# rrwick/Autocycler

Hardware: AMD Instinct MI355X
Metric: Mbp/sec through compress->unitig GFA (k=51) (higher is better)
Workload: dtype u64

## Files before the change

### autocycler_amd/csrc/device_prims.hpp

```cpp
#pragma once

namespace ac {

#ifdef AC_EMU
inline u64 state_load(const u64* p) {
    struct Seen { const u64* p; u64 v; u32 n; };
    static thread_local Seen seen[1024];
    Seen& e = seen[wv::tid() & 1023u];
    const u64 v = *p;
    if (e.p == p && e.v == v) { if (++e.n > (1u << 20)) { e.n = 0; throw DeviceError("lockstep emulation: a look-back waits for a tile state that is never published"); } }
    else { e.p = p; e.v = v; e.n = 0; }
    return v;
}
inline void state_store(u64* p, u64 v) { *p = v; }
#else
__device__ inline u64 state_load(const u64* p) { return __hip_atomic_load(p, __ATOMIC_RELAXED, __HIP_MEMORY_SCOPE_AGENT); }
__device__ inline void state_store(u64* p, u64 v) { __hip_atomic_store(p, v, __ATOMIC_RELAXED, __HIP_MEMORY_SCOPE_AGENT); }
#endif

AC_HD int prim_popc64(u64 x) {
#if defined(__HIP_DEVICE_COMPILE__)
    return __popcll(x);
#else
    return __builtin_popcountll(x);
// ... 38 lines not shown
            AC_HIP_CHECK(hipStreamSynchronize(0));
            if (want != cap) { if (words) (void)hipFree(words); AC_HIP_CHECK(hipMalloc((void**)&words, want * 8)); }
            AC_HIP_CHECK(hipMemset(words, 0, want * 8));
#endif
            cap = want; epoch = 0; tickets = 0;
        }
        *epoch_out = ++epoch;
        *ticket_base = tickets;
        tickets += tiles;
    }
};
enum { CTX_SCANPOOL = 7 };
inline ScanPool& scan_pool() { return ctx_object<ScanPool>(CTX_SCANPOOL); }

template <class T, int OP, bool INCL>
AC_KERNEL void __launch_bounds__(256) scan_kernel(const T* in, T* out, u64 n, u64* pool, u64 epoch, u64 ticket_base) {
    AC_SHARED u64 s_wave[4];
    AC_SHARED u64 s_prefix;
    AC_SHARED u64 s_tile;
    u64* state = pool + 1;
    const unsigned tid = wv::tid();
    const int lane = wv::lane(), wave = (int)(tid >> 6);
    if (tid == 0) s_tile = atomic_add64(&pool[0], 1) - ticket_base;
    wv::block_sync();
    const u64 tile = s_tile;
    const u64 base = tile * SCAN_TILE + (u64)tid * SCAN_ITEMS;
    alignas(16) T v[SCAN_ITEMS];
    if (base + SCAN_ITEMS <= n && (((uintptr_t)(in + base)) & 15u) == 0) {
        const PrimV16* p = (const PrimV16*)(in + base);
        PrimV16* q = (PrimV16*)v;
#pragma unroll
        for (u32 j = 0; j < SCAN_ITEMS * sizeof(T) / 16; j++) q[j] = p[j];
    } else {
#pragma unroll
        for (u32 j = 0; j < SCAN_ITEMS; j++) v[j] = base + j < n ? in[base + j] : (T)0;
    }
    u64 tsum = 0;
#pragma unroll
    for (u32 j = 0; j < SCAN_ITEMS; j++) tsum = scan_op<OP>(tsum, (u64)v[j]);
    u64 incl = tsum;
// ... 28 lines not shown
        }
        if (lane == 0) s_prefix = excl;
    }
    wv::block_sync();
    u64 run = scan_op<OP>(s_prefix, wave_off);
    {
        const u64 before = wave_shfl_up64(incl, 1);
        if (lane > 0) run = scan_op<OP>(run, before);
    }
    alignas(16) T o[SCAN_ITEMS];
#pragma unroll
    for (u32 j = 0; j < SCAN_ITEMS; j++) {
        const u64 nxt = scan_op<OP>(run, (u64)v[j]);
        o[j] = (T)(INCL ? nxt : run);
        run = nxt;
    }
    if (base + SCAN_ITEMS <= n && (((uintptr_t)(out + base)) & 15u) == 0) {
        PrimV16* q = (PrimV16*)(out + base);
        const PrimV16* p = (const PrimV16*)o;
#pragma unroll
        for (u32 j = 0; j < SCAN_ITEMS * sizeof(T) / 16; j++) q[j] = p[j];
    } else {
#pragma unroll
        for (u32 j = 0; j < SCAN_ITEMS; j++) if (base + j < n) out[base + j] = o[j];
    }
}
template <class T, int OP, bool INCL> inline void scan_launch(const T* in, T* out, size_t n, stream_t s) {
    if (!n) return;
    if (s != 0) throw DeviceError("scan: stream 0 only (the state pool's tickets are stream-ordered)");
    const u64 tiles = (n + SCAN_TILE - 1) / SCAN_TILE;
    u64 epoch = 0, ticket_base = 0;
    ScanPool& pool = scan_pool();
    pool.take(tiles, &epoch, &ticket_base);
    launch_wave_kernel(scan_kernel<T, OP, INCL>, tiles, s, in, out, (u64)n, pool.words, epoch, ticket_base);
}
inline void inclusive_scan_u32(const u32* in, u32* out, size_t n, stream_t s = 0) { scan_launch<u32, SCAN_ADD, true>(in, out, n, s); }
inline void inclusive_max_scan_u32(const u32* in, u32* out, size_t n, stream_t s = 0) { scan_launch<u32, SCAN_MAX, true>(in, out, n, s); }
inline void exclusive_scan_u32(const u32* in, u32* out, size_t n, stream_t s = 0) { scan_launch<u32, SCAN_ADD, false>(in, out, n, s); }
inline void exclusive_scan_u64(const u64* in, u64* out, size_t n, stream_t s = 0) { scan_launch<u64, SCAN_ADD, false>(in, out, n, s); }

static const u32 RS_ITEMS = 8, RS_TILE = 256 * RS_ITEMS, RS_MAX_PASSES = 8;
static const int RS_LB = 16;
template <int UNUSED> AC_KERNEL void __launch_bounds__(256) radix_hist_kernel(const u64* keys, u64 n, int passes, int begin_bit, int end_bit, u32* hist) {
    AC_SHARED u32 s_hist[RS_MAX_PASSES * 256];
    const unsigned tid = wv::tid();
    for (int i = (int)tid; i < passes * 256; i += 256) s_hist[i] = 0;
    wv::block_sync();
    const u64 base = (u64)wv::bid() * RS_TILE;
    for (u32 j = 0; j < RS_ITEMS; j++) {
        const u64 i = base + (u64)j * 256 + tid;
// ... 228 lines not shown
```

### autocycler_amd/csrc/device_rt.hpp

```cpp
#pragma once
#include <cstdio>
#include <cstdlib>
#include <cstring>
#include <stdexcept>
#include <string>
#include <vector>
#include <algorithm>

#include <mutex>
#include <time.h>
#include <unistd.h>

#include "kmer_ops.hpp"
#include "graph_types.hpp"
#include "wave_rt.hpp"

#ifndef AC_EMU
#include <hip/hip_runtime.h>
#endif

namespace ac {

struct DeviceError : std::runtime_error { using std::runtime_error::runtime_error; };
struct NeedExactPositions {};
// ... 464 lines not shown
    if (s == 0) flush_fills();
    if (use_mailbox() && bytes <= Mailbox::CAP) {
        MailItem it{d, (u32)bytes, 0};
        Mailbox::get().fetch(&it, &h, 1, s);
        return;
    }
    static const bool use_scratch = getenv("AC_NO_PINNED_SCRATCH") == nullptr;
    if (use_scratch && bytes <= (64 << 10)) {
        void* p = pinned_scratch(bytes);
        rt_counters().readbacks++;
        AC_HIP_CHECK(hipMemcpyAsync(p, d, bytes, hipMemcpyDeviceToHost, s));
        AC_HIP_CHECK(hipStreamSynchronize(s));
        memcpy(h, p, bytes);
        return;
    }
#endif
    copy_d2h_async(h, d, bytes, s);
#ifndef AC_EMU
    AC_HIP_CHECK(hipStreamSynchronize(s));
#endif
}
class ReadBatch {
  public:
    void add(void* h, const void* d, size_t bytes) { if (bytes) items_.push_back(Item{h, d, bytes}); }
    void run(stream_t s = 0) {
#ifdef AC_EMU
        for (auto& it : items_) memcpy(it.h, it.d, it.bytes);
        (void)s;
#else
        size_t total = 0;
        for (auto& it : items_) total += (it.bytes + 63) & ~(size_t)63;
        if (total == 0) return;
        if (s == 0) flush_fills();
        if (use_mailbox() && total <= Mailbox::CAP && items_.size() <= (size_t)MAIL_MAX_ITEMS) {
            MailItem mi[MAIL_MAX_ITEMS]; void* dst[MAIL_MAX_ITEMS];
            size_t o = 0;
            for (size_t i = 0; i < items_.size(); i++) { mi[i] = MailItem{items_[i].d, (u32)items_[i].bytes, (u32)o}; dst[i] = items_[i].h; o += (items_[i].bytes + 63) & ~(size_t)63; }
            Mailbox::get().fetch(mi, dst, (int)items_.size(), s);
            items_.clear();
            return;
        }
// ... 193 lines not shown
    for (u64 b0 = 0; b0 < blocks; b0 += 0xFFFFFFu)
        wv::launch_kernel(+[](const F* g, u64 nn, u64 base) { const u64 tid = base + (u64)wv::bid() * 256 + wv::tid(); (*g)(tid, tid < nn); },
                          (unsigned)std::min<u64>(0xFFFFFFu, blocks - b0), 256u, fp, n, b0 * 256);
#else
    const u64 blocks = (n + 255) / 256;
    if (s == 0) flush_fills();
    if (debug_launch()) debug_launch_note<F>(n, false);
    for (u64 b0 = 0; b0 < blocks; b0 += MAX_LAUNCH_BLOCKS) {
        rt_counters().launches++;
        hipLaunchKernelGGL(functor_kernel_full<F>, dim3((unsigned)std::min(MAX_LAUNCH_BLOCKS, blocks - b0)), dim3(256), 0, s, n, f, b0 * 256);
        AC_HIP_CHECK(hipGetLastError());
    }
    if (debug_launch()) debug_launch_note<F>(n, true);
#endif
}
template <class K, class... A> void launch_wave_kernel_sized(K kernel, u64 blocks, unsigned threads, stream_t s, A... args) {
    if (blocks == 0) return;
    if (blocks > 0xFFFFFFULL) throw DeviceError("grid too large");
#ifdef AC_EMU
    (void)s;
    wv::launch_kernel(kernel, (unsigned)blocks, threads, args...);
#else
    if (s == 0) flush_fills();
    rt_counters().launches++;
    hipLaunchKernelGGL(kernel, dim3((unsigned)blocks), dim3(threads), 0, s, args...);
    AC_HIP_CHECK(hipGetLastError());
#endif
}
template <class K, class... A> void launch_wave_kernel(K kernel, u64 blocks, stream_t s, A... args) { launch_wave_kernel_sized(kernel, blocks, 256u, s, args...); }
AC_D u32 wave_alloc32(u32* counter, u32 amount) {
// ... 21 lines not shown
```

### autocycler_amd/csrc/graph_impl.hpp

```cpp
#pragma once
#include "graph_build.hpp"

#include <chrono>
#include <cmath>
#include <map>
#include <string>
#include <algorithm>
#include <atomic>
#include <thread>
#include <functional>
#include <condition_variable>
#include <mutex>
#include <fcntl.h>
#include <unistd.h>
#if defined(__x86_64__)
#include <immintrin.h>
#endif

#include "device_rt.hpp"

namespace ac {

static double now_s() {
    return std::chrono::duration<double>(std::chrono::steady_clock::now().time_since_epoch()).count();
// ... 269 lines not shown
    bool shard_degree_flags;
    bool insert_adaptive;
    u64 insert_growth;
    u64 insert_waves_target;
    bool renum_two_pass;
    u32 renum_max_group;
    u32 path_chunk_env;
    long upload_threads_env;
    bool debug_arena;
    bool degree_diag;
    int multi_transport;
    int multi_fragments;
    int multi_tail;
    u64 trim_batch_bytes;
    u64 resolve_batch_bytes;
    static Knobs read() {
        Knobs k;
        k.minkey_variant = [&]() -> int { const char* e = getenv("AC_MINKEY_VARIANT"); return e ? atoi(e) : -1; }();
        k.path_copy = [&]() -> int { const char* e = getenv("AC_PATH_COPY"); return e ? (atoi(e) != 0 ? 1 : 0) : 2; }();
        k.run_piece = [&]() -> u64 { const char* e = getenv("AC_RUN_PIECE"); const long v = e ? atol(e) : 0; return v > 0 ? (u64)v : 4096; }();
        k.pos_cap = [&]() -> u32 { const char* e = getenv("AC_POS_CAP"); const long v = e ? atol(e) : 65536; return v < 0 ? 0u : (u32)std::min<long>(v, 0x3FFFFFFF); }();
        k.path_filter = [&]() -> bool { const char* e = getenv("AC_PATH_FILTER"); return e ? atoi(e) != 0 : true; }();
        k.host_remap_mode = [&]() -> int { const char* e = getenv("AC_HOST_REMAP"); return e ? (atoi(e) == 2 ? 2 : (atoi(e) != 0 ? 1 : 0)) : -1; }();
        k.remap_block = [&]() -> u32 { const char* e = getenv("AC_REMAP_BLOCK"); int v = e ? atoi(e) : 4096; v = v < 64 ? 64 : (v > 65536 ? 65536 : v); return (u32)(v & ~63); }();
        k.minkey_prefix_bases = [&]() -> int { const char* e = getenv("AC_MINKEY_PREFIX_BASES"); int v = e ? atoi(e) : 31; return v < 1 ? 1 : (v > 31 ? 31 : v); }();
        k.seed_prefix_sort = [&]() -> bool { const char* e = getenv("AC_SEED_PREFIX_SORT"); return e ? atoi(e) != 0 : true; }();
        k.seed_max_group = [&]() -> u32 { const char* e = getenv("AC_SEED_MAX_GROUP"); int v = e ? atoi(e) : 1024; return (u32)(v < 1 ? 1 : v); }();
        k.seed_prefix_bits = [&]() -> int { const char* e = getenv("AC_SEED_PREFIX_BITS"); if (!e) return 0; int v = atoi(e); return v < 1 ? 1 : (v > 64 ? 64 : v); }();
        k.degree_region_cap = [&]() -> u32 { const char* e = getenv("AC_DEGREE_REGION_CAP"); int v = e ? atoi(e) : 0; return (u32)(v < 0 ? 0 : v); }();
        k.upload_direct_mode = [&]() -> int { const char* e = getenv("AC_UPLOAD_DIRECT"); return e ? (atoi(e) != 0 ? 1 : 0) : -1; }();
// ... 21 lines not shown
        k.shard_degree_flags = [&]() -> bool { const char* e = getenv("AC_SHARD_DEGREE_FLAGS"); return e ? atoi(e) != 0 : true; }();
        k.insert_adaptive = [&]() -> bool { const char* e = getenv("AC_INSERT_ADAPT"); return e ? atoi(e) != 0 : true; }();
        k.insert_growth = [&]() -> u64 { const char* e = getenv("AC_INSERT_GROWTH"); long x = e ? atol(e) : 2; return (u64)(x < 2 ? 2 : x); }();
        k.insert_waves_target = [&]() -> u64 { const char* e = getenv("AC_INSERT_WAVES"); long x = e ? atol(e) : 16384; return (u64)(x < 1024 ? 1024 : x); }();
        k.renum_two_pass = [&]() -> bool { const char* e = getenv("AC_RENUM_TWO_PASS"); return e && atoi(e) != 0; }();
        k.renum_max_group = [&]() -> u32 { const char* e = getenv("AC_RENUM_MAX_GROUP"); int v = e ? atoi(e) : 64; return (u32)(v < 1 ? 1 : (v > 64 ? 64 : v)); }();
        k.path_chunk_env = [&]() -> u32 { const char* e = getenv("AC_PATH_CHUNK"); if (!e) return 0; int v = atoi(e); return (u32)(v < 64 ? 64 : (v > 4096 ? 4096 : v)); }();
        k.upload_threads_env = [&]() -> long { const char* e = getenv("AC_UPLOAD_THREADS"); return e ? atol(e) : 24; }();
        k.debug_arena = [&]() -> bool { return getenv("AC_DEBUG_ARENA") != nullptr; }();
        k.degree_diag = [&]() -> bool { return getenv("AC_DEGREE_DIAG") != nullptr; }();
        k.multi_transport = [&]() -> int { const char* e = getenv("AC_MULTI_TRANSPORT"); return !e ? 0 : (!strcmp(e, "host") ? 1 : (!strcmp(e, "rccl") ? 2 : 0)); }();
        k.multi_fragments = [&]() -> int { const char* e = getenv("AC_MULTI_FRAGMENTS"); return e && !strcmp(e, "bytes") ? 1 : 0; }();
        k.multi_tail = [&]() -> int { const char* e = getenv("AC_MULTI_TAIL"); return e && !strcmp(e, "replicated") ? 1 : 0; }();
        k.trim_batch_bytes = [&]() -> u64 { const char* e = getenv("AC_TRIM_BATCH_BYTES"); const long long v = e ? atoll(e) : 0; return v > 0 ? (u64)v : (u64)4 << 30; }();
        k.resolve_batch_bytes = [&]() -> u64 { const char* e = getenv("AC_RESOLVE_BATCH_BYTES"); const long long v = e ? atoll(e) : 0; return v > 0 ? (u64)v : (u64)1 << 30; }();
        return k;
    }
};
const Knobs& knobs();
void knobs_refresh();

[[maybe_unused]] static int minkey_variant() { return knobs().minkey_variant; }
[[maybe_unused]] static int path_copy() { return knobs().path_copy; }
[[maybe_unused]] static bool path_copy_pays(u64 n_text, u32 assemblies, u32 k, double r2) {
    const double A = (double)std::max<u32>(assemblies, 1);
    const double entries = (double)n_text * std::min(1.0, 2.0 * A * r2 / (double)k);
    const double saving = entries * 53e-12 * std::max(0.0, 1.0 - 2.0 / A), cost = 0.25e-3 + 0.3e-12 * (double)n_text;
    return saving > 1.5 * cost;
}
[[maybe_unused]] static u64 run_piece() { return knobs().run_piece; }
// ... 147 lines not shown
    void begin(BuildTimings* t) {
        tm = t; t_begin = t0 = now_s();
        rt_counters() = RtCounters();
        host_remap_allowed = false;
        counters.alloc(8); counters.fill_bytes(0);
        sort_flags.alloc(2); sort_flags.fill_bytes(0);
    }
    void check_sizes(const PackedText& t) const {
        if (t.n_text >= POS_MASK) throw DeviceError("input too large for 40-bit text positions");
        if (t.n_seqs == 0 || t.n_text < (u64)k + 2) throw DeviceError("no sequences");
    }
    template <int W> void insert(const PackedText& t, u32 hint, DBuf<u64>* slots_out, u64* cap_out, u64* n_distinct_out, DBuf<u64>* bm_out, bool want_sib = false);
    DBuf<u64> sflags;
    DBuf<u64> runs; DBuf<u32> run_count; u64 run_rows = 0, run_rows_cap = 0;
    DBuf<u64> loc_bm; DBuf<u32> loc_wprefix; bool local_insert_of_shard = false;
    struct CopyPlan { bool ok = false; u64 R = 0, NW = 0, Rb = 0; DBuf<RunRec> rr; DBuf<u32> rseq; DBuf<u64> wfirst, w_begin, w_end; DBuf<u32> w_gap; } cplan;
    void occupancy_bitmap(const DBuf<u64>& sl, u64 c, DBuf<u64>* occ_out, const u64* sflags_in, u64* sib_out, stream_t s = 0);
    DBuf<u64> occ;
    DBuf<u64> sib;
    DBuf<u64> sibn; bool sib_pending = false;
    DBuf<u32> kcontrib, pend, pidx; u64 n_pending = 0, n_first = 0;
    DBuf<u64> endset, endset_bloom; u64 endset_mask = 0;
    u32 n_owners = 1, my_owner = 0;
    void* upload_done = nullptr; u64 upload_avail = 0; bool upload_pending = false;
    struct UploadJob {
#ifndef AC_EMU
        const std::vector<SeqView>* seqs = nullptr;
        std::vector<uint64_t> off;
        uint32_t k = 0; u64 n = 0, CH = 0, SUB = 0, n_chunks = 0, slot_bytes = 0; int NSLOT = 0, dev = 0;
        hipStream_t up = nullptr, pk = nullptr;
        u64* d_bits = nullptr;
// ... 136 lines not shown
```

### autocycler_amd/csrc/graph_stages.hip

```cpp
#include "graph_impl.hpp"

namespace ac {

template <int W>
void GraphBuilder::Impl::insert(const PackedText& pt, u32 hint, DBuf<u64>* slots_out, u64* cap_out, u64* n_distinct_out, DBuf<u64>* bm_out, bool want_sib) {
    TextCtx t = pt.ctx((int)k);
    const u64 p_end_all = pt.n_text - (u64)k + 1;
    if (hint == 0) hint = 1;
    u64 est = pt.n_bases / hint;
    u64 c = next_pow2(std::max<u64>(1024, est * 3 + 4096));
    if (&pt == &uni && distinct_upper) {
        const u64 mine = distinct_upper / std::max<u32>(n_owners, 1) + distinct_upper / (8 * (u64)std::max<u32>(n_owners, 1)) + 4096;
        c = next_pow2(std::max<u64>(1024, mine * 10 / 7));
    }
    if (c > next_pow2(pt.n_bases * 2 + 1024)) c = next_pow2(pt.n_bases * 2 + 1024);
    const int shift = table_shift() >= 0 ? table_shift() : (c > (1ULL << 25) ? 0 : 1);
    c <<= shift;
    struct CapMemo { u64 n_text = 0, cap = 0; u32 k = 0; int shift = -2; u32 owners = 0; };
    static thread_local CapMemo memo[4]; static thread_local unsigned memo_next = 0;
    const u32 memo_owners = (&pt == &uni) ? n_owners : 1u;
    for (const CapMemo& m : memo)
        if (pt.n_text == m.n_text && k == m.k && m.shift == table_shift() && m.owners == memo_owners && m.cap > c) c = m.cap;
    const int copy_mode = (&pt == &loc && (want_sib || (local_insert_of_shard && shard_path_copy()))) ? path_copy() : 0;
    bool want_runs = false;
// ... 439 lines not shown
    std::vector<u64> h_first = to_host(first, n_shards);
    u64 end = n_queries;
    for (u32 o = n_shards; o-- > 0;) {
        if (h_first[o] == ~0ULL) { counts_host[o] = 0; continue; }
        counts_host[o] = end - h_first[o];
        end = h_first[o];
    }
}
template <int W> void GraphBuilder::Impl::answer_queries(const u64* d_keys, u64 n, u64* d_out) {
    launch(n, AnswerFunctor<W>{G->ctx((int)k), graph_table(), d_keys, d_out});
}

template <int W> bool GraphBuilder::Impl::walk_copy_prepare(u32 PC, const Novel& nv_text) {
    TextCtx t = loc.ctx((int)k);
    cplan = CopyPlan();
    const Arena::Mark mk = Arena::device().mark();
    DBuf<u32> rfirst(run_rows + 1);
    exclusive_scan_u32(run_count.ptr(), rfirst.ptr(), run_rows + 1);
    const u64 R0 = read_scalar(rfirst.ptr() + run_rows);
    if (R0 == 0 || R0 >= 0xFFFFFFF0ULL) { Arena::device().rewind(mk); return false; }
    DBuf<RunRec> sorted(R0);
    launch(run_rows * RUN_ROW, RunGatherFunctor{runs.ptr(), run_count.ptr(), rfirst.ptr(), sorted.ptr()});
    DBuf<u32> ok(R0 + 1), at(R0 + 1); DBuf<u64> covered(1, true); DBuf<u32> overlap(1, true);
    ok.fill_bytes(0);
    DBuf<RunRec> fixed(R0); DBuf<u32> fseq(R0);
    launch(R0, RunFilterFunctor{sorted.ptr(), fixed.ptr(), R0, nv_text, loc.n_text, ok.ptr(), covered.ptr(), t, overlap.ptr(), run_piece(), fseq.ptr()});
    exclusive_scan_u32(ok.ptr(), at.ptr(), R0 + 1);
    const u64 Rb = R0 + loc.n_text / run_piece() + 1;
    CopyPlan& c = cplan;
    c.rr.alloc(Rb); c.rseq.alloc(Rb);
    launch(R0, RunCompactFunctor{fixed.ptr(), ok.ptr(), at.ptr(), c.rr.ptr(), run_piece(), fseq.ptr(), c.rseq.ptr(), nv_text, loc.n_text});
    DBuf<u64> gw(Rb + 2);
    c.wfirst.alloc(Rb + 2);
    launch(Rb + 2, GapWalkersFunctor{c.rr.ptr(), at.ptr() + R0, loc.n_text, PC, gw.ptr()});
    exclusive_scan_u64(gw.ptr(), c.wfirst.ptr(), Rb + 2);
    u64 h_cov = 0, NW = 0; u32 h_R = 0, h_overlap = 0;
    { ReadBatch rb; rb.add(&h_cov, covered.ptr(), 8); rb.add(&h_R, at.ptr() + R0, 4); rb.add(&h_overlap, overlap.ptr(), 4); rb.add(&NW, c.wfirst.ptr() + (Rb + 1), 8); rb.run(); }
    const u64 R = h_R;
    if (knobs().debug_arena) fprintf(stderr, "path copy: %llu runs on the list, %llu pieces usable, covering %llu of %llu positions, %llu walkers\n", (unsigned long long)R0, (unsigned long long)R, (unsigned long long)h_cov, (unsigned long long)loc.n_text, (unsigned long long)NW);
    if (R == 0 || h_overlap || h_cov * 2 < loc.n_text || NW == 0 || NW >= 0xFFFFFFF0ULL) {
        cplan = CopyPlan();
        Arena::device().rewind(mk);
        return false;
    }
    c.w_begin.alloc(NW); c.w_end.alloc(NW); c.w_gap.alloc(NW);
    launch(NW, WalkerRangeFunctor{c.rr.ptr(), R, loc.n_text, PC, c.wfirst.ptr(), c.w_begin.ptr(), c.w_end.ptr(), c.w_gap.ptr()});
    c.R = R; c.NW = NW; c.Rb = Rb; c.ok = true;
    return true;
}
template <int W> void GraphBuilder::Impl::walk_copy_finish(u32 PC) {
    TextCtx t = loc.ctx((int)k), g = G->ctx((int)k);
    Table tb = graph_table();
    Novel nv{bm.ptr(), wprefix.ptr()};
    UnitigCtx uc{head.ptr(), scan.ptr(), rank.ptr(), uorient.ptr(), ustart.ptr(), ulen.ptr(), U, N};
    CopyPlan& c = cplan;
    const u64 R = c.R, NW = c.NW;
    DBuf<u64> wcount(NW + 1), woff(NW + 1);
    const u64 n_slots = ((NW + 63) / 64) * 64 * PC;
    DBuf<int32_t> stage(n_slots); DBuf<u16> stage_off(n_slots);
    DBuf<u32> seq_tid(loc.n_seqs), seq_j(loc.n_seqs);
    wcount.fill_bytes(0);
    const bool filter = maybe_dest_valid;
    walk_tables(filter);
    walked_plain = false;
    DBuf<V16> uinfo(U);
    launch(U, WalkInfoFunctor{uc, filter ? maybe_dest.ptr() : nullptr, uinfo.ptr()});
    launch(NW, PathWalkFunctor<W>{t, g, tb, nv, uc, uinfo.ptr(), wl_text.ptr(), PC, stage.ptr(), wcount.ptr(), seq_tid.ptr(), seq_j.ptr(),
                                 depth_u.ptr(), minpos_fwd_u.ptr(), minpos_rev_u.ptr(), counters.ptr() + 4, filter ? maybe_dest.ptr() : nullptr,
                                 pos_cap_now, 0, walk_answers, NW, c.w_begin.ptr(), c.w_end.ptr(), stage_off.ptr(), nullptr, nullptr});
    exclusive_scan_u64(wcount.ptr(), woff.ptr(), NW + 1);
    const u64 NE = read_scalar(woff.ptr() + NW);
    DBuf<int32_t> ent(NE); DBuf<u64> ent_pos(NE), ent_end(NE); DBuf<u8> ent_want(NE); DBuf<u32> ent_gap(NE);
    launch_full(NW, WalkCompactFunctor{stage.ptr(), stage_off.ptr(), wcount.ptr(), woff.ptr(), c.w_begin.ptr(), c.w_gap.ptr(), PC, NW, uinfo.ptr(),
                                       ent.ptr(), ent_pos.ptr(), ent_end.ptr(), ent_want.ptr(), ent_gap.ptr()});
    DBuf<u64> ra(R), rcnt(R + 1), seg(2 * R + 2), segoff(2 * R + 2); DBuf<u32> cov(NE + 1), copies(NE + 1);
    cov.fill_bytes(0);
    launch(R, RunRangeFunctor{c.rr.ptr(), ent_pos.ptr(), ent_end.ptr(), NE, ra.ptr(), rcnt.ptr(), cov.ptr()});
    launch(2 * R + 2, SegCountFunctor{c.wfirst.ptr(), woff.ptr(), rcnt.ptr(), R, seg.ptr()});
    exclusive_scan_u64(seg.ptr(), segoff.ptr(), 2 * R + 2);
    inclusive_scan_u32(cov.ptr(), copies.ptr(), NE + 1);
    n_ent = read_scalar(segoff.ptr() + (2 * R + 1));
    if (knobs().debug_arena) {
        std::vector<u64> h = to_host(rcnt, R); u64 mx = 0, sum = 0, big = 0, hist[8] = {0};
        for (u64 v : h) { mx = std::max(mx, v); sum += v; if (v > 256) big++; int b = 0; while ((32ull << b) < v && b < 7) b++; hist[b]++; }
        fprintf(stderr, "path copy: %llu pieces, entries per piece: max %llu, mean %.1f, %llu above 256; hist(<=32,64,128,..): %llu %llu %llu %llu %llu %llu %llu %llu\n", (unsigned long long)R, (unsigned long long)mx, (double)sum / (double)R, (unsigned long long)big,
                (unsigned long long)hist[0], (unsigned long long)hist[1], (unsigned long long)hist[2], (unsigned long long)hist[3], (unsigned long long)hist[4], (unsigned long long)hist[5], (unsigned long long)hist[6], (unsigned long long)hist[7]);
    }
    ent_val.alloc(n_ent);
    int32_t* const out_ptr = ent_val.ptr();
    launch(NE, GapOutFunctor{ent.ptr(), ent_gap.ptr(), woff.ptr(), c.wfirst.ptr(), segoff.ptr(), copies.ptr(), out_ptr, depth_u.ptr()});
    launch_full(R * 32, RunOutFunctor<32, 1>{c.rr.ptr(), R, ra.ptr(), rcnt.ptr(), segoff.ptr(), ent.ptr(), ent_pos.ptr(), ent_end.ptr(), uinfo.ptr(),
                                             ent_want.ptr(), t, c.rseq.ptr(), minpos_fwd_u.ptr(), minpos_rev_u.ptr(), out_ptr, pos_cap_now});
    launch(loc.n_seqs, PathOffCopyFunctor{seq_tid.ptr(), seq_j.ptr(), woff.ptr(), c.wfirst.ptr(), c.w_gap.ptr(), segoff.ptr(), path_off.ptr()});
    tm->n_path_entries = n_ent;
    tm->path_runs_copied = R; tm->path_entries_walked = NE;
    copy_h2d(path_off.ptr() + loc.n_seqs, &n_ent, 8);
    launch(loc.n_seqs, PathEndsFunctor{ent_val.ptr(), path_off.ptr(), fs0.ptr(), fe0.ptr(), rank.ptr(), uorient.ptr()});
    walk_to_seed_order();
}

template <int W> void GraphBuilder::Impl::walk() {
// ... 70 lines not shown
```

### autocycler_amd/csrc/kernels_paths.inc

```
AC_HD u32 idx_of(int32_t v) { return (u32)(v < 0 ? -v : v) - 1; }
struct MaybeDestFunctor {
    const int32_t* links; u8* maybe;
    AC_HD static u64 row(int32_t v) { return ((u64)((u32)(v < 0 ? -v : v) - 1) * 2 + (v > 0 ? 0 : 1)) * 5; }
    AC_HD void operator()(u64 idx) const {
        const u32 x = (u32)(idx >> 1);
        const bool inputs = (idx & 1) == 0;
        const int32_t xnum = (int32_t)x + 1;
        const u64 mine = row(inputs ? -xnum : xnum);
        u32 n = 0;
        bool ok = true;
        for (int c = 0; c < 5; c++) {
            int32_t p = links[mine + (u64)c];
            if (p == 0) continue;
            n++;
            int32_t other = inputs ? -p : p;
            const u64 theirs = row(inputs ? other : -other);
            u32 m = 0; int32_t only = 0;
            for (int d = 0; d < 5; d++) { int32_t q = links[theirs + (u64)d]; if (q != 0) { m++; only = q; } }
            if (!(m == 1 && only == (inputs ? xnum : -xnum))) ok = false;
            if ((u32)(other < 0 ? -other : other) - 1 == x) ok = false;
        }
        maybe[idx] = (ok && n >= 2) ? 1 : 0;
    }
};
// ... 165 lines not shown
        for (u32 o0 = 0; o0 < total; o0 += 64) {
            const u32 o = o0 + (u32)lane;
            int lo = 0;
#pragma unroll
            for (int step = 32; step; step >>= 1) {
                const int cand = lo + step;
                const u32 v = (u32)wv::shfl((int)rel, cand & 63);
                if (cand < 64 && v <= o) lo = cand;
            }
            const u32 start = (u32)wv::shfl((int)rel, lo);
            if (o < total) ent_val[base + o] = rows[(u64)(o - start) * 64 + (u64)lo];
        }
    }
};
struct RunRec { u64 p; u64 n; u64 q; };
struct RunGatherFunctor {
    const u64* runs; const u32* count; const u32* rfirst; RunRec* out;
    AC_HD void operator()(u64 tid) const {
        const u64 row = tid / RUN_ROW; const u32 i = (u32)(tid % RUN_ROW);
        if (i >= count[row]) return;
        const u64* rec = runs + 3 * tid;
        out[(u64)rfirst[row] + i] = RunRec{rec[0], rec[1], rec[2]};
    }
};
AC_HD bool run_piece_good(const Novel& nv, u64 n_text, const RunRec& x, u64 d, u64 n) {
    const bool same = (x.q >> 63) != 0;
    const u64 q = x.q & ~(1ULL << 63);
    if (!same && q < d + n - 1) return false;
    const u64 qlo = same ? q + d : q - d + 1 - n, qhi = qlo + n;
    if (qhi > n_text) return false;
    return (u64)(novel_rank(nv, qhi) - novel_rank(nv, qlo)) == n;
}
struct RunFilterFunctor {
    const RunRec* runs; RunRec* fixed; u64 n_runs; Novel nv; u64 n_text; u32* ok; u64* covered; TextCtx t; u32* overlap; u64 piece; u32* fseq;
    AC_D void operator()(u64 r) const {
        RunRec x = runs[r];
        const bool same = (x.q >> 63) != 0;
        u64 q = x.q & ~(1ULL << 63);
        u32 lo = 0;
        {
            u32 hi = t.n_seqs;
            while (hi - lo > 1) { u32 mid = lo + ((hi - lo) >> 1); if (t.seq_off[mid] <= x.p) lo = mid; else hi = mid; }
            if (t.n_seqs && t.seq_off[lo] == x.p && x.n > 0) {
                x.p += 1; x.n -= 1; q = same ? q + 1 : q - 1;
                x.q = q | ((u64)(same ? 1 : 0) << 63);
            }
        }
        fixed[r] = x; fseq[r] = lo;
        if (r > 0 && runs[r - 1].p + runs[r - 1].n > runs[r].p) atomic_or32(overlap, 1u);
// ... 13 lines not shown
        if (!ok[r]) return;
        const RunRec x = runs[r];
        const bool same = (x.q >> 63) != 0;
        const u64 q = x.q & ~(1ULL << 63);
        u32 j = 0;
        for (u64 d = 0; d < x.n; d += piece) {
            const u64 n = x.n - d < piece ? x.n - d : piece;
            if (!run_piece_good(nv, n_text, x, d, n)) continue;
            out[at[r] + j] = RunRec{x.p + d, n, (same ? q + d : q - d) | ((u64)(same ? 1 : 0) << 63)};
            rseq[at[r] + j] = fseq[r];
            j++;
        }
    }
};
struct GapWalkersFunctor {
    const RunRec* runs; const u32* n_runs_at; u64 n_text; u32 pc; u64* n_walkers;
    AC_HD void operator()(u64 g) const {
        const u64 n_runs = *n_runs_at;
        if (g > n_runs) { n_walkers[g] = 0; return; }
        const u64 b = g == 0 ? 0 : runs[g - 1].p + runs[g - 1].n, e = g == n_runs ? n_text : runs[g].p;
        n_walkers[g] = e > b ? (e - b + pc - 1) / pc : 0;
    }
};
struct WalkerRangeFunctor {
    const RunRec* runs; u64 n_runs; u64 n_text; u32 pc; const u64* wfirst; u64* w_begin; u64* w_end; u32* w_gap;
    AC_HD void operator()(u64 w) const {
        u64 lo = 0, hi = n_runs + 1;
        while (hi - lo > 1) { u64 mid = lo + ((hi - lo) >> 1); if (wfirst[mid] <= w) lo = mid; else hi = mid; }
        const u64 g = lo;
        const u64 b = g == 0 ? 0 : runs[g - 1].p + runs[g - 1].n, e = g == n_runs ? n_text : runs[g].p;
        const u64 wb = b + (w - wfirst[g]) * (u64)pc;
// ... 34 lines not shown
            const u64 wb = (u64)wv::shfl64((unsigned long long)my_begin, lo);
            const u32 gap = (u32)wv::shfl((int)my_gap, lo);
            if (o < total) {
                const u64 slot = row0 + (u64)(o - start) * 64 + (u64)lo;
                put(base + o, stage[slot], wb + (u64)stage_off[slot], gap);
            }
        }
    }
};
AC_HD u64 lower_bound_u64(const u64* a, u64 n, u64 key) {
    u64 lo = 0, hi = n;
    while (lo < hi) { const u64 mid = lo + ((hi - lo) >> 1); if (a[mid] < key) lo = mid + 1; else hi = mid; }
    return lo;
}
struct RunRangeFunctor {
    const RunRec* runs; const u64* ent_pos; const u64* ent_end; u64 n_ent; u64* ra; u64* cnt; u32* cov;
    AC_D void operator()(u64 r) const {
        const RunRec x = runs[r];
        const bool same = (x.q >> 63) != 0;
        const u64 q = x.q & ~(1ULL << 63);
        u64 a, b;
        if (same) { a = lower_bound_u64(ent_pos, n_ent, q); const u64 m = n_ent - a < x.n ? n_ent - a : x.n; b = a + lower_bound_u64(ent_pos + a, m, q + x.n); }
        else { a = lower_bound_u64(ent_end, n_ent, q + 1 - x.n); const u64 m = n_ent - a < x.n ? n_ent - a : x.n; b = a + lower_bound_u64(ent_end + a, m, q + 1); }
        ra[r] = a; cnt[r] = b - a;
        if (b > a) { atomic_add32(&cov[a], 1u); atomic_add32(&cov[b], 0xFFFFFFFFu); }
    }
};
struct SegCountFunctor {
    const u64* wfirst; const u64* woff; const u64* run_cnt; u64 n_runs; u64* seg;
    AC_HD void operator()(u64 i) const {
        if (i > 2 * n_runs) { seg[i] = 0; return; }
        if (i & 1) { seg[i] = run_cnt[i >> 1]; return; }
        const u64 g = i >> 1;
        seg[i] = woff[wfirst[g + 1]] - woff[wfirst[g]];
    }
};
struct GapOutFunctor {
    const int32_t* ent; const u32* ent_gap; const u64* woff; const u64* wfirst; const u64* segoff; const u32* copies; int32_t* out; u32* depth;
    AC_D void operator()(u64 e) const {
        const u64 g = ent_gap[e];
        const int32_t v = ent[e];
        out[segoff[2 * g] + (e - woff[wfirst[g]])] = v;
// ... 123 lines not shown
```

Before: 88040.

## Replace host read-backs in walk copy planning with device-bounded launches

Sizes the walk-copy plan arrays from host-known upper bounds and passes the actual counts to kernels and scans through device pointers, so the grid-stride launches and scans no longer need those counts on the host. Several scalar read-backs in walk_copy_prepare are merged into one batched read, and the entry count in walk_copy_finish is read together with n_ent instead of on its own. The aim is to remove host-device synchronisation stalls. In exchange, arrays are over-allocated to the bound when arena headroom allows, and some kernels launch more blocks than they need and exit early.

```diff
diff --git a/autocycler_amd/csrc/device_prims.hpp b/autocycler_amd/csrc/device_prims.hpp
--- a/autocycler_amd/csrc/device_prims.hpp
+++ b/autocycler_amd/csrc/device_prims.hpp
@@ -76,7 +76,7 @@
 inline ScanPool& scan_pool() { return ctx_object<ScanPool>(CTX_SCANPOOL); }
 
 template <class T, int OP, bool INCL>
-AC_KERNEL void __launch_bounds__(256) scan_kernel(const T* in, T* out, u64 n, u64* pool, u64 epoch, u64 ticket_base) {
+AC_KERNEL void __launch_bounds__(256) scan_kernel(const T* in, T* out, u64 n, u64* pool, u64 epoch, u64 ticket_base, const u64* n_dev, u64 n_extra, u64* total_out) {
     AC_SHARED u64 s_wave[4];
     AC_SHARED u64 s_prefix;
     AC_SHARED u64 s_tile;
@@ -86,6 +86,8 @@
     if (tid == 0) s_tile = atomic_add64(&pool[0], 1) - ticket_base;
     wv::block_sync();
     const u64 tile = s_tile;
+    if (n_dev) n = bounded_count(n, *n_dev, n_extra);
+    if (tile * SCAN_TILE >= n) return;
     const u64 base = tile * SCAN_TILE + (u64)tid * SCAN_ITEMS;
     alignas(16) T v[SCAN_ITEMS];
     if (base + SCAN_ITEMS <= n && (((uintptr_t)(in + base)) & 15u) == 0) {
@@ -144,6 +146,7 @@
         const u64 nxt = scan_op<OP>(run, (u64)v[j]);
         o[j] = (T)(INCL ? nxt : run);
         run = nxt;
+        if (total_out && base + j + 1 == n) *total_out = nxt;
     }
     if (base + SCAN_ITEMS <= n && (((uintptr_t)(out + base)) & 15u) == 0) {
         PrimV16* q = (PrimV16*)(out + base);
@@ -162,8 +165,19 @@
     u64 epoch = 0, ticket_base = 0;
     ScanPool& pool = scan_pool();
     pool.take(tiles, &epoch, &ticket_base);
-    launch_wave_kernel(scan_kernel<T, OP, INCL>, tiles, s, in, out, (u64)n, pool.words, epoch, ticket_base);
-}
+    launch_wave_kernel(scan_kernel<T, OP, INCL>, tiles, s, in, out, (u64)n, pool.words, epoch, ticket_base, (const u64*)nullptr, (u64)0, (u64*)nullptr);
+}
+template <class T, int OP, bool INCL> inline void scan_launch_bounded(const T* in, T* out, size_t bound, const u64* d_count, u64 extra, u64* total_out) {
+    if (!bound) return;
+    const u64 tiles = (bound + SCAN_TILE - 1) / SCAN_TILE;
+    u64 epoch = 0, ticket_base = 0;
+    ScanPool& pool = scan_pool();
+    pool.take(tiles, &epoch, &ticket_base);
+    launch_wave_kernel(scan_kernel<T, OP, INCL>, tiles, 0, in, out, (u64)bound, pool.words, epoch, ticket_base, d_count, extra, total_out);
+}
+inline void exclusive_scan_u32_bounded(const u32* in, u32* out, size_t bound, const u64* d_count, u64 extra = 0, u64* total_out = nullptr) { scan_launch_bounded<u32, SCAN_ADD, false>(in, out, bound, d_count, extra, total_out); }
+inline void exclusive_scan_u64_bounded(const u64* in, u64* out, size_t bound, const u64* d_count, u64 extra = 0, u64* total_out = nullptr) { scan_launch_bounded<u64, SCAN_ADD, false>(in, out, bound, d_count, extra, total_out); }
+inline void inclusive_scan_u32_bounded(const u32* in, u32* out, size_t bound, const u64* d_count, u64 extra = 0, u64* total_out = nullptr) { scan_launch_bounded<u32, SCAN_ADD, true>(in, out, bound, d_count, extra, total_out); }
 inline void inclusive_scan_u32(const u32* in, u32* out, size_t n, stream_t s = 0) { scan_launch<u32, SCAN_ADD, true>(in, out, n, s); }
 inline void inclusive_max_scan_u32(const u32* in, u32* out, size_t n, stream_t s = 0) { scan_launch<u32, SCAN_MAX, true>(in, out, n, s); }
 inline void exclusive_scan_u32(const u32* in, u32* out, size_t n, stream_t s = 0) { scan_launch<u32, SCAN_ADD, false>(in, out, n, s); }
diff --git a/autocycler_amd/csrc/device_rt.hpp b/autocycler_amd/csrc/device_rt.hpp
--- a/autocycler_amd/csrc/device_rt.hpp
+++ b/autocycler_amd/csrc/device_rt.hpp
@@ -502,6 +502,8 @@
         memcpy(h, p, bytes);
         return;
     }
+#else
+    if (bytes <= ((size_t)64 << 10)) rt_counters().readbacks++;
 #endif
     copy_d2h_async(h, d, bytes, s);
 #ifndef AC_EMU
@@ -513,6 +515,7 @@
     void add(void* h, const void* d, size_t bytes) { if (bytes) items_.push_back(Item{h, d, bytes}); }
     void run(stream_t s = 0) {
 #ifdef AC_EMU
+        if (!items_.empty()) rt_counters().readbacks++;
         for (auto& it : items_) memcpy(it.h, it.d, it.bytes);
         (void)s;
 #else
@@ -736,6 +739,54 @@
     if (debug_launch()) debug_launch_note<F>(n, true);
 #endif
 }
+AC_HD u64 bounded_count(u64 bound, u64 count, u64 extra) {
+    if (count >= bound) return bound;
+    return extra < bound - count ? count + extra : bound;
+}
+inline bool walk_entries_fit(u64 bound, u64 item_bytes, u64 arrays, u64 headroom) {
+    const u64 slack = arrays * 256;
+    if (bound >= 0xFFFFFFF0ULL || headroom <= slack) return false;
+    return bound + 1 <= (headroom - slack) / item_bytes;
+}
+#ifndef AC_EMU
+static const u64 BOUNDED_MAX_BLOCKS = 4096;
+template <class F>
+__global__ void __launch_bounds__(256) functor_kernel_bounded(u64 bound, const u64* d_count, u64 extra, F f) {
+    const u64 n = bounded_count(bound, *d_count, extra), stride = (u64)gridDim.x * 256;
+    for (u64 i = (u64)blockIdx.x * 256 + threadIdx.x; i < n; i += stride) f(i);
+}
+template <class F>
+__global__ void __launch_bounds__(256) functor_kernel_full_bounded(u64 bound, const u64* d_count, u64 extra, F f) {
+    const u64 n = bounded_count(bound, *d_count, extra), stride = (u64)gridDim.x * 256;
+    for (u64 b = (u64)blockIdx.x * 256; b < n; b += stride) f(b + threadIdx.x, b + threadIdx.x < n);
+}
+#endif
+template <class F> void launch_bounded(u64 bound, const u64* d_count, const F& f, u64 extra = 0, stream_t s = 0) {
+    if (bound == 0) return;
+#ifdef AC_EMU
+    launch(bounded_count(bound, *d_count, extra), f, s);
+#else
+    if (s == 0) flush_fills();
+    if (debug_launch()) debug_launch_note<F>(bound, false);
+    rt_counters().launches++;
+    hipLaunchKernelGGL(functor_kernel_bounded<F>, dim3((unsigned)std::min(BOUNDED_MAX_BLOCKS, (bound + 255) / 256)), dim3(256), 0, s, bound, d_count, extra, f);
+    AC_HIP_CHECK(hipGetLastError());
+    if (debug_launch()) debug_launch_note<F>(bound, true);
+#endif
+}
+template <class F> void launch_full_bounded(u64 bound, const u64* d_count, const F& f, u64 extra = 0, stream_t s = 0) {
+    if (bound == 0) return;
+#ifdef AC_EMU
+    launch_full(bounded_count(bound, *d_count, extra), f, s);
+#else
+    if (s == 0) flush_fills();
+    if (debug_launch()) debug_launch_note<F>(bound, false);
+    rt_counters().launches++;
+    hipLaunchKernelGGL(functor_kernel_full_bounded<F>, dim3((unsigned)std::min(BOUNDED_MAX_BLOCKS, (bound + 255) / 256)), dim3(256), 0, s, bound, d_count, extra, f);
+    AC_HIP_CHECK(hipGetLastError());
+    if (debug_launch()) debug_launch_note<F>(bound, true);
+#endif
+}
 template <class K, class... A> void launch_wave_kernel_sized(K kernel, u64 blocks, unsigned threads, stream_t s, A... args) {
     if (blocks == 0) return;
     if (blocks > 0xFFFFFFULL) throw DeviceError("grid too large");
diff --git a/autocycler_amd/csrc/graph_impl.hpp b/autocycler_amd/csrc/graph_impl.hpp
--- a/autocycler_amd/csrc/graph_impl.hpp
+++ b/autocycler_amd/csrc/graph_impl.hpp
@@ -307,6 +307,7 @@
     int multi_tail;
     u64 trim_batch_bytes;
     u64 resolve_batch_bytes;
+    long walk_headroom_mb;
     static Knobs read() {
         Knobs k;
         k.minkey_variant = [&]() -> int { const char* e = getenv("AC_MINKEY_VARIANT"); return e ? atoi(e) : -1; }();
@@ -358,6 +359,7 @@
         k.multi_tail = [&]() -> int { const char* e = getenv("AC_MULTI_TAIL"); return e && !strcmp(e, "replicated") ? 1 : 0; }();
         k.trim_batch_bytes = [&]() -> u64 { const char* e = getenv("AC_TRIM_BATCH_BYTES"); const long long v = e ? atoll(e) : 0; return v > 0 ? (u64)v : (u64)4 << 30; }();
         k.resolve_batch_bytes = [&]() -> u64 { const char* e = getenv("AC_RESOLVE_BATCH_BYTES"); const long long v = e ? atoll(e) : 0; return v > 0 ? (u64)v : (u64)1 << 30; }();
+        k.walk_headroom_mb = [&]() -> long { const char* e = getenv("AC_WALK_HEADROOM_MB"); return e ? std::max<long>(atol(e), 0) : -1; }();
         return k;
     }
 };
@@ -535,7 +537,8 @@
     DBuf<u64> sflags;
     DBuf<u64> runs; DBuf<u32> run_count; u64 run_rows = 0, run_rows_cap = 0;
     DBuf<u64> loc_bm; DBuf<u32> loc_wprefix; bool local_insert_of_shard = false;
-    struct CopyPlan { bool ok = false; u64 R = 0, NW = 0, Rb = 0; DBuf<RunRec> rr; DBuf<u32> rseq; DBuf<u64> wfirst, w_begin, w_end; DBuf<u32> w_gap; } cplan;
+    struct CopyPlan { bool ok = false; u64 R = 0, NW = 0, Rb = 0, ne_bound = 0;
+                      DBuf<RunRec> rr; DBuf<u32> rseq; DBuf<u64> wfirst, w_begin, w_end; DBuf<u32> w_gap; } cplan;
     void occupancy_bitmap(const DBuf<u64>& sl, u64 c, DBuf<u64>* occ_out, const u64* sflags_in, u64* sib_out, stream_t s = 0);
     DBuf<u64> occ;
     DBuf<u64> sib;
diff --git a/autocycler_amd/csrc/graph_stages.hip b/autocycler_amd/csrc/graph_stages.hip
--- a/autocycler_amd/csrc/graph_stages.hip
+++ b/autocycler_amd/csrc/graph_stages.hip
@@ -477,39 +477,46 @@
 template <int W> bool GraphBuilder::Impl::walk_copy_prepare(u32 PC, const Novel& nv_text) {
     TextCtx t = loc.ctx((int)k);
     cplan = CopyPlan();
+    const u64 R0b = run_rows * RUN_ROW, Rb = R0b + loc.n_text / run_piece() + 1;
+    if (Rb >= 0xFFFFFFF0ULL) return false;
     const Arena::Mark mk = Arena::device().mark();
     DBuf<u32> rfirst(run_rows + 1);
+    DBuf<u64> plan(PLAN_WORDS, true);
     exclusive_scan_u32(run_count.ptr(), rfirst.ptr(), run_rows + 1);
-    const u64 R0 = read_scalar(rfirst.ptr() + run_rows);
-    if (R0 == 0 || R0 >= 0xFFFFFFF0ULL) { Arena::device().rewind(mk); return false; }
-    DBuf<RunRec> sorted(R0);
-    launch(run_rows * RUN_ROW, RunGatherFunctor{runs.ptr(), run_count.ptr(), rfirst.ptr(), sorted.ptr()});
-    DBuf<u32> ok(R0 + 1), at(R0 + 1); DBuf<u64> covered(1, true); DBuf<u32> overlap(1, true);
-    ok.fill_bytes(0);
-    DBuf<RunRec> fixed(R0); DBuf<u32> fseq(R0);
-    launch(R0, RunFilterFunctor{sorted.ptr(), fixed.ptr(), R0, nv_text, loc.n_text, ok.ptr(), covered.ptr(), t, overlap.ptr(), run_piece(), fseq.ptr()});
-    exclusive_scan_u32(ok.ptr(), at.ptr(), R0 + 1);
-    const u64 Rb = R0 + loc.n_text / run_piece() + 1;
+    const u64* d_R0 = plan.ptr() + PLAN_R0;
+    DBuf<RunRec> sorted(R0b);
+    launch(R0b, RunGatherFunctor{runs.ptr(), run_count.ptr(), rfirst.ptr(), sorted.ptr(), run_rows, plan.ptr()});
+    DBuf<u32> ok(R0b), at(R0b);
+    DBuf<RunRec> fixed(R0b); DBuf<u32> fseq(R0b);
+    launch_bounded(R0b, d_R0, RunFilterFunctor{sorted.ptr(), fixed.ptr(), nv_text, loc.n_text, ok.ptr(), plan.ptr() + PLAN_COVERED, t, (u32*)(plan.ptr() + PLAN_OVERLAP), run_piece(), fseq.ptr()});
+    exclusive_scan_u32_bounded(ok.ptr(), at.ptr(), R0b, d_R0, 0, plan.ptr() + PLAN_R);
     CopyPlan& c = cplan;
     c.rr.alloc(Rb); c.rseq.alloc(Rb);
-    launch(R0, RunCompactFunctor{fixed.ptr(), ok.ptr(), at.ptr(), c.rr.ptr(), run_piece(), fseq.ptr(), c.rseq.ptr(), nv_text, loc.n_text});
+    launch_bounded(R0b, d_R0, RunCompactFunctor{fixed.ptr(), ok.ptr(), at.ptr(), c.rr.ptr(), run_piece(), fseq.ptr(), c.rseq.ptr(), nv_text, loc.n_text});
     DBuf<u64> gw(Rb + 2);
     c.wfirst.alloc(Rb + 2);
-    launch(Rb + 2, GapWalkersFunctor{c.rr.ptr(), at.ptr() + R0, loc.n_text, PC, gw.ptr()});
-    exclusive_scan_u64(gw.ptr(), c.wfirst.ptr(), Rb + 2);
-    u64 h_cov = 0, NW = 0; u32 h_R = 0, h_overlap = 0;
-    { ReadBatch rb; rb.add(&h_cov, covered.ptr(), 8); rb.add(&h_R, at.ptr() + R0, 4); rb.add(&h_overlap, overlap.ptr(), 4); rb.add(&NW, c.wfirst.ptr() + (Rb + 1), 8); rb.run(); }
-    const u64 R = h_R;
-    if (knobs().debug_arena) fprintf(stderr, "path copy: %llu runs on the list, %llu pieces usable, covering %llu of %llu positions, %llu walkers\n", (unsigned long long)R0, (unsigned long long)R, (unsigned long long)h_cov, (unsigned long long)loc.n_text, (unsigned long long)NW);
-    if (R == 0 || h_overlap || h_cov * 2 < loc.n_text || NW == 0 || NW >= 0xFFFFFFF0ULL) {
+    launch_bounded(Rb + 2, plan.ptr() + PLAN_R, GapWalkersFunctor{c.rr.ptr(), plan.ptr() + PLAN_R, loc.n_text, PC, gw.ptr()}, 2);
+    exclusive_scan_u64_bounded(gw.ptr(), c.wfirst.ptr(), Rb + 2, plan.ptr() + PLAN_R, 2, plan.ptr() + PLAN_NW);
+    u64 h_plan[PLAN_WORDS];
+    { ReadBatch rb; rb.add(h_plan, plan.ptr(), sizeof h_plan); rb.run(); }
+    const u64 R0 = h_plan[PLAN_R0], R = h_plan[PLAN_R], NW = h_plan[PLAN_NW], h_cov = h_plan[PLAN_COVERED];
+    const bool h_overlap = (u32)h_plan[PLAN_OVERLAP] != 0;
+    if (R0 > R0b || R > Rb) throw DeviceError("internal error: more followed runs than their rows hold");
+    if (knobs().debug_arena) fprintf(stderr, "path copy: %llu runs on the list (room for %llu), %llu pieces usable, covering %llu of %llu positions, %llu walkers\n", (unsigned long long)R0, (unsigned long long)R0b, (unsigned long long)R, (unsigned long long)h_cov, (unsigned long long)loc.n_text, (unsigned long long)NW);
+    if (R0 == 0 || R == 0 || h_overlap || h_cov * 2 < loc.n_text || NW == 0 || NW >= 0xFFFFFFF0ULL) {
         cplan = CopyPlan();
         Arena::device().rewind(mk);
         return false;
     }
     c.w_begin.alloc(NW); c.w_end.alloc(NW); c.w_gap.alloc(NW);
     launch(NW, WalkerRangeFunctor{c.rr.ptr(), R, loc.n_text, PC, c.wfirst.ptr(), c.w_begin.ptr(), c.w_end.ptr(), c.w_gap.ptr()});
-    c.R = R; c.NW = NW; c.Rb = Rb; c.ok = true;
+    c.R = R; c.NW = NW; c.Rb = Rb; c.ne_bound = loc.n_text - h_cov; c.ok = true;
     return true;
+}
+static u64 walk_arena_headroom() {
+    if (knobs().walk_headroom_mb >= 0) return (u64)knobs().walk_headroom_mb << 20;
+    const Arena& a = Arena::device();
+    return a.capacity() - a.total_used();
 }
 template <int W> void GraphBuilder::Impl::walk_copy_finish(u32 PC) {
     TextCtx t = loc.ctx((int)k), g = G->ctx((int)k);
@@ -532,22 +539,31 @@
                                  depth_u.ptr(), minpos_fwd_u.ptr(), minpos_rev_u.ptr(), counters.ptr() + 4, filter ? maybe_dest.ptr() : nullptr,
                                  pos_cap_now, 0, walk_answers, NW, c.w_begin.ptr(), c.w_end.ptr(), stage_off.ptr(), nullptr, nullptr});
     exclusive_scan_u64(wcount.ptr(), woff.ptr(), NW + 1);
-    const u64 NE = read_scalar(woff.ptr() + NW);
-    DBuf<int32_t> ent(NE); DBuf<u64> ent_pos(NE), ent_end(NE); DBuf<u8> ent_want(NE); DBuf<u32> ent_gap(NE);
+    const u64* d_NE = woff.ptr() + NW;
+    static const u64 ENTRY_BYTES = sizeof(int32_t) + 2 * sizeof(u64) + sizeof(u8) + sizeof(u32) + 2 * sizeof(u32);
+    const u64 ne_bound = c.ne_bound;
+    const bool bounded = walk_entries_fit(ne_bound, ENTRY_BYTES, 7, walk_arena_headroom());
+    u64 NE = bounded ? ne_bound : read_scalar(d_NE);
+    const u64 ne_cap = NE;
+    DBuf<int32_t> ent(ne_cap); DBuf<u64> ent_pos(ne_cap), ent_end(ne_cap); DBuf<u8> ent_want(ne_cap); DBuf<u32> ent_gap(ne_cap);
     launch_full(NW, WalkCompactFunctor{stage.ptr(), stage_off.ptr(), wcount.ptr(), woff.ptr(), c.w_begin.ptr(), c.w_gap.ptr(), PC, NW, uinfo.ptr(),
                                        ent.ptr(), ent_pos.ptr(), ent_end.ptr(), ent_want.ptr(), ent_gap.ptr()});
-    DBuf<u64> ra(R), rcnt(R + 1), seg(2 * R + 2), segoff(2 * R + 2); DBuf<u32> cov(NE + 1), copies(NE + 1);
-    cov.fill_bytes(0);
-    launch(R, RunRangeFunctor{c.rr.ptr(), ent_pos.ptr(), ent_end.ptr(), NE, ra.ptr(), rcnt.ptr(), cov.ptr()});
+    DBuf<u64> ra(R), rcnt(R + 1), seg(2 * R + 2), segoff(2 * R + 2); DBuf<u32> cov(ne_cap + 1), copies(ne_cap + 1);
+    if (bounded) launch_bounded(ne_cap + 1, d_NE, ZeroU32Functor{cov.ptr()}, 1);
+    else cov.fill_bytes(0);
+    launch(R, RunRangeFunctor{c.rr.ptr(), ent_pos.ptr(), ent_end.ptr(), d_NE, ra.ptr(), rcnt.ptr(), cov.ptr()});
     launch(2 * R + 2, SegCountFunctor{c.wfirst.ptr(), woff.ptr(), rcnt.ptr(), R, seg.ptr()});
     exclusive_scan_u64(seg.ptr(), segoff.ptr(), 2 * R + 2);
-    inclusive_scan_u32(cov.ptr(), copies.ptr(), NE + 1);
-    n_ent = read_scalar(segoff.ptr() + (2 * R + 1));
+    if (bounded) inclusive_scan_u32_bounded(cov.ptr(), copies.ptr(), ne_cap + 1, d_NE, 1);
+    else inclusive_scan_u32(cov.ptr(), copies.ptr(), NE + 1);
+    { ReadBatch rb; rb.add(&n_ent, segoff.ptr() + (2 * R + 1), 8); rb.add(&NE, d_NE, 8); rb.run(); }
+    if (NE > ne_cap) throw DeviceError("internal error: the gap walkers emitted more path entries than their gaps have positions");
     if (knobs().debug_arena) {
         std::vector<u64> h = to_host(rcnt, R); u64 mx = 0, sum = 0, big = 0, hist[8] = {0};
         for (u64 v : h) { mx = std::max(mx, v); sum += v; if (v > 256) big++; int b = 0; while ((32ull << b) < v && b < 7) b++; hist[b]++; }
         fprintf(stderr, "path copy: %llu pieces, entries per piece: max %llu, mean %.1f, %llu above 256; hist(<=32,64,128,..): %llu %llu %llu %llu %llu %llu %llu %llu\n", (unsigned long long)R, (unsigned long long)mx, (double)sum / (double)R, (unsigned long long)big,
                 (unsigned long long)hist[0], (unsigned long long)hist[1], (unsigned long long)hist[2], (unsigned long long)hist[3], (unsigned long long)hist[4], (unsigned long long)hist[5], (unsigned long long)hist[6], (unsigned long long)hist[7]);
+        fprintf(stderr, "path copy: %llu entries walked, arrays for %llu (%s)\n", (unsigned long long)NE, (unsigned long long)ne_cap, bounded ? "the bound: no read-back" : "read back");
     }
     ent_val.alloc(n_ent);
     int32_t* const out_ptr = ent_val.ptr();
diff --git a/autocycler_amd/csrc/kernels_paths.inc b/autocycler_amd/csrc/kernels_paths.inc
--- a/autocycler_amd/csrc/kernels_paths.inc
+++ b/autocycler_amd/csrc/kernels_paths.inc
@@ -203,9 +203,11 @@
     }
 };
 struct RunRec { u64 p; u64 n; u64 q; };
+enum { PLAN_R0 = 0, PLAN_R, PLAN_NW, PLAN_COVERED, PLAN_OVERLAP, PLAN_WORDS };
 struct RunGatherFunctor {
-    const u64* runs; const u32* count; const u32* rfirst; RunRec* out;
+    const u64* runs; const u32* count; const u32* rfirst; RunRec* out; u64 n_rows; u64* plan;
     AC_HD void operator()(u64 tid) const {
+        if (tid == 0) plan[PLAN_R0] = rfirst[n_rows];
         const u64 row = tid / RUN_ROW; const u32 i = (u32)(tid % RUN_ROW);
         if (i >= count[row]) return;
         const u64* rec = runs + 3 * tid;
@@ -221,7 +223,7 @@
     return (u64)(novel_rank(nv, qhi) - novel_rank(nv, qlo)) == n;
 }
 struct RunFilterFunctor {
-    const RunRec* runs; RunRec* fixed; u64 n_runs; Novel nv; u64 n_text; u32* ok; u64* covered; TextCtx t; u32* overlap; u64 piece; u32* fseq;
+    const RunRec* runs; RunRec* fixed; Novel nv; u64 n_text; u32* ok; u64* covered; TextCtx t; u32* overlap; u64 piece; u32* fseq;
     AC_D void operator()(u64 r) const {
         RunRec x = runs[r];
         const bool same = (x.q >> 63) != 0;
@@ -265,7 +267,7 @@
     }
 };
 struct GapWalkersFunctor {
-    const RunRec* runs; const u32* n_runs_at; u64 n_text; u32 pc; u64* n_walkers;
+    const RunRec* runs; const u64* n_runs_at; u64 n_text; u32 pc; u64* n_walkers;
     AC_HD void operator()(u64 g) const {
         const u64 n_runs = *n_runs_at;
         if (g > n_runs) { n_walkers[g] = 0; return; }
@@ -330,8 +332,9 @@
     return lo;
 }
 struct RunRangeFunctor {
-    const RunRec* runs; const u64* ent_pos; const u64* ent_end; u64 n_ent; u64* ra; u64* cnt; u32* cov;
+    const RunRec* runs; const u64* ent_pos; const u64* ent_end; const u64* n_ent_at; u64* ra; u64* cnt; u32* cov;
     AC_D void operator()(u64 r) const {
+        const u64 n_ent = *n_ent_at;
         const RunRec x = runs[r];
         const bool same = (x.q >> 63) != 0;
         const u64 q = x.q & ~(1ULL << 63);
@@ -342,6 +345,7 @@
         if (b > a) { atomic_add32(&cov[a], 1u); atomic_add32(&cov[b], 0xFFFFFFFFu); }
     }
 };
+struct ZeroU32Functor { u32* a; AC_HD void operator()(u64 i) const { a[i] = 0; } };
 struct SegCountFunctor {
     const u64* wfirst; const u64* woff; const u64* run_cnt; u64 n_runs; u64* seg;
     AC_HD void operator()(u64 i) const {
```

Measured after the change: 85660. -2.7%, worse.
